# abacusorg/abacusutils

Hardware: AMD Instinct MI355X
Metric: halos/sec HOD populate (higher is better)
Workload: dtype f64; 1 GPU; C2: 1e+07 synthetic halos + 1e+07 subsample particles per GPU (seed 600+rank), LRG HOD of tests/abacus_hod.yaml:31-47, rsd=True, catalog resident in HBM; n_halo=10000000, n_part=10000000, n_gal=107980, enable_ranks=False

## Files before the change

abacusutils_amd/csrc/hod.hip:

```cpp
#include <cmath>
#include <cstring>
#include <cstddef>
#include <vector>

#include "../../include/abacus_hip.h"
#include "common.hpp"
#include "hod_classify.hpp"
#include "hod_envelope.hpp"

namespace abacus {
int exclusive_scan_u32(unsigned int *counters, int64_t n, int64_t *out, DevBuf &scratch, int zero_counters);
int sort_pairs_u16(const unsigned short *keys_in, unsigned short *keys_out, const unsigned int *val_in, unsigned int *val_out,
                   int64_t n, DevBuf &tmp);
}
using namespace abacus;

namespace {

constexpr int TILE = 2048;
constexpr int BLOCK = 256;
constexpr int PER_THREAD = TILE / BLOCK;
constexpr int SB_TILES_SPARSE = 16, SB_TILES_DENSE = 8;
constexpr int SB_TILES_MIN = 8, SB_TILES_MAX = 16;

// ... 739 lines not shown
    asm volatile("global_load_dwordx4 %0, %1, off" : "=v"(dst) : "v"(p) : "memory");
}
__device__ __forceinline__ void aload_u16(unsigned int &dst, const void *p) {
    asm volatile("global_load_ushort %0, %1, off" : "=v"(dst) : "v"(p) : "memory");
}
__device__ __forceinline__ void aload_i8(int &dst, const void *p) {
    asm volatile("global_load_sbyte %0, %1, off" : "=v"(dst) : "v"(p) : "memory");
}
template <int K>
__device__ __forceinline__ void await_vm() {
    asm volatile("s_waitcnt vmcnt(%0)" ::"n"(K) : "memory");
}
__device__ __forceinline__ void touch4(v4u &a) { asm volatile("" : "+v"(a)); }
__device__ __forceinline__ void touch1(unsigned int &a) { asm volatile("" : "+v"(a)); }
__device__ __forceinline__ void touch1i(int &a) { asm volatile("" : "+v"(a)); }

struct ExactCand {
    double mass, w, rnd, dc, fe, sh, r0, r1, r2, r3;
    long long pinds;
    int q, loc;
};

__device__ __forceinline__ void fetch_cand(const HodPtrs &a, const abacus_hod_params &p, bool sat, int64_t i, bool need_ranks,
                                           bool need_conf, ExactCand &c) {
    c.r0 = c.r1 = c.r2 = c.r3 = 1.0;
    c.pinds = 0;
    if (!sat) {
        if (a.hrec) {
            const HaloRec &r = a.hrec[i];
            c.mass = r.mass, c.w = r.multis, c.rnd = r.rnd, c.dc = r.deltac, c.fe = r.fenv, c.sh = p.want_ELG ? r.shear : 0.0;
        } else {
            c.rnd = a.hrandoms[i];
            c.mass = a.hmass[i], c.w = a.hmultis[i], c.dc = load1(a.hdeltac, i, 0.0), c.fe = load1(a.hfenv, i, 0.0),
            c.sh = p.want_ELG ? load1(a.hshear, i, 0.0) : 0.0;
        }
    } else {
        if (a.prec) {
            const PartRec &r = a.prec[i];
            c.mass = r.mass, c.w = r.weights, c.rnd = r.rnd, c.dc = r.deltac, c.fe = r.fenv, c.sh = p.want_ELG ? r.shear : 0.0;
            if (need_ranks) c.r0 = r.rank0, c.r1 = r.rank1, c.r2 = r.rank2, c.r3 = r.rank3;
            if (need_conf) c.pinds = r.pinds;
        } else {
            if (need_conf) c.pinds = a.pinds[i];
            c.rnd = a.prandoms[i];
            c.mass = a.phmass[i], c.w = a.pweights[i], c.dc = load1(a.pdeltac, i, 0.0), c.fe = load1(a.pfenv, i, 0.0),
            c.sh = p.want_ELG ? load1(a.pshear, i, 0.0) : 0.0;
            if (need_ranks) c.r0 = a.pranks[i], c.r1 = a.pranksv[i], c.r2 = a.pranksp[i], c.r3 = a.pranksr[i];
        }
    }
}

template <int lane>
__device__ __forceinline__ unsigned int writelane_u32(unsigned int v, unsigned int old) {
#if defined(__HIP_DEVICE_COMPILE__)
    asm("v_writelane_b32 %0, %1, %2" : "+v"(old) : "s"(v), "n"(lane));
#endif
    return old;
}

template <int XB, bool PIPE, int SBT, int SRC = 0, bool MASKS = true>
__device__ __forceinline__ void hod_exact_body(const HodPtrs &a, int first_sb, const abacus_hod_params &p, const SatPre &pre,
                                               const abacus_cls::ClsConst &cc, int use_cls, int clear_prev,
                                               const SbIndex *sx = nullptr) {
    static_assert(SRC == 0 || (!PIPE && XB >= 128 && SBT * TILE <= 65536), "the key index feeds the plain form");
    static_assert(SRC == 1 || MASKS, "only the key index form may leave the keep masks alone");
    constexpr int SB_TILES = SBT, SB_OBJ = SBT * TILE, SB_WORDS = SB_OBJ / 32;
    constexpr int WORDS_PER_THREAD = SB_WORDS / XB;
    static_assert(SB_WORDS % XB == 0 && XB <= 512 && SB_OBJ <= 65536, "bitmap words must divide over the workgroup");
    __shared__ ExactLds<SBT> L;
    __shared__ abacus_hod_params s_p;
    __shared__ SatPre s_pre;
    const int tid = threadIdx.x;
    static_assert(sizeof(abacus_hod_params) % 8 == 0 && sizeof(SatPre) % 8 == 0, "copied as 8-byte words");
    if (tid < (int)(sizeof(abacus_hod_params) / 8))
        reinterpret_cast<unsigned long long *>(&s_p)[tid] = reinterpret_cast<const unsigned long long *>(&p)[tid];
    if (tid < (int)(sizeof(SatPre) / 8))
        reinterpret_cast<unsigned long long *>(&s_pre)[tid] = reinterpret_cast<const unsigned long long *>(&pre)[tid];
    const int g = (int)blockIdx.x + first_sb;
    const bool sat = g >= a.nsb_c;
    const int S = sat ? g - a.nsb_c : g;
// ... 73 lines not shown
            int lo = 0, hi = SBX_BINS - 1;
            while (lo < hi) {
                const int mid = (lo + hi + 1) >> 1;
                if (s_bpre[mid] <= j) lo = mid;
                else hi = mid - 1;
            }
            const int l = ((sat ? sx->sidx_s : sx->sidx_c) + obj_first)[(int)s_bstart[lo] + (j - s_bpre[lo])];
            q = l / TILE, loc = l % TILE;
        } else {
            q = exact_find_tile(L, j);
            loc = queue[(int64_t)(tile_first + q) * TILE + (j - L.pre[q])];
        }
    };
    auto fetch = [&](int q, int loc, ExactCand &c) {
        c.q = q, c.loc = loc;
        fetch_cand(a, p, sat, (int64_t)(tile_first + q) * TILE + loc, need_ranks, need_conf, c);
    };
    auto classify = [&](const ExactCand &c, int kc) {
        if (!use_cls) return -1;
        return sat ? abacus_cls::sat_classify(cc, c.mass, c.w, c.rnd, c.dc, c.fe, c.sh, c.r0, c.r1, c.r2, c.r3, kc)
                   : abacus_cls::cent_classify(cc, c.mass, c.w, c.rnd, c.dc, c.fe, c.sh);
    };
    auto exact_chain = [&](const ExactCand &c, int kc) {
        return sat ? sat_decide_cold(&s_p, &s_pre, c.mass, c.w, c.rnd, c.dc, c.fe, c.sh, c.r0, c.r1, c.r2, c.r3, kc)
                   : cent_decide_cold(&s_p, c.mass, c.w, c.rnd, c.dc, c.fe, c.sh);
    };
    auto record = [&](const ExactCand &c, int kk) {
        if (kk) {
            if constexpr (MASKS) (sat ? a.keep_s : a.keep_c)[(int64_t)(tile_first + c.q) * TILE + c.loc] = (int8_t)kk;
            const int ls = c.q * TILE + c.loc;
            atomicOr(&L.bm[kk - 1][ls >> 5], 1u << (ls & 31));
// ... 7 lines not shown
            fetch(q, loc, c);
            const int kc = need_conf ? a.keep_c[c.pinds] : 0;
            int kk = classify(c, kc);
            if (kk < 0) kk = exact_chain(c, kc);
            record(c, kk);
        }
    } else {
        const char *rec = sat ? reinterpret_cast<const char *>(a.prec) : reinterpret_cast<const char *>(a.hrec);
        const int64_t rb = sat ? (int64_t)sizeof(PartRec) : (int64_t)sizeof(HaloRec);
        auto queue_addr = [&](int jj, int &q) {
            jj = min(jj, total - 1);
            q = exact_find_tile(L, jj);
            return queue + ((int64_t)(tile_first + q) * TILE + (jj - L.pre[q]));
        };
        auto rec_addr = [&](int q, int loc) { return rec + ((int64_t)(tile_first + q) * TILE + loc) * rb; };
        auto decode = [&](const v4u (&r)[6], int q, int loc, ExactCand &c) {
            auto dbl = [](unsigned int lo, unsigned int hi) { return __hiloint2double((int)hi, (int)lo); };
            c.q = q, c.loc = loc;
            c.mass = dbl(r[0].x, r[0].y), c.w = dbl(r[0].z, r[0].w), c.rnd = dbl(r[1].x, r[1].y), c.dc = dbl(r[1].z, r[1].w);
            c.fe = dbl(r[2].x, r[2].y), c.sh = p.want_ELG ? dbl(r[2].z, r[2].w) : 0.0;
            c.r0 = c.r1 = c.r2 = c.r3 = 1.0;
            c.pinds = 0;
            if (sat) {
                if (need_ranks) c.r0 = dbl(r[3].x, r[3].y), c.r1 = dbl(r[3].z, r[3].w), c.r2 = dbl(r[4].x, r[4].y), c.r3 = dbl(r[4].z, r[4].w);
                c.pinds = (long long)(((unsigned long long)r[5].y << 32) | r[5].x);
            }
        };
        if (total > 0) {
            int j = tid;
            int q0, q1, q2;
            unsigned int loc0, loc1, loc2 = 0;
            v4u raw[6];
            aload_u16(loc0, queue_addr(j, q0));
            aload_u16(loc1, queue_addr(j + XB, q1));
            await_vm<0>();
            touch1(loc0), touch1(loc1);
            {
                const char *r0 = rec_addr(q0, (int)loc0);
#pragma unroll
                for (int l = 0; l < 6; l++)
                    if (l < 3 || sat) aload16(raw[l], r0 + 16 * l);
            }
            await_vm<0>();
#pragma unroll
            for (int l = 0; l < 6; l++)
                if (l < 3 || sat) touch4(raw[l]);
            ExactCand cur;
            decode(raw, q0, (int)loc0, cur);
            int kc = 0;
            if (need_conf) {
                aload_i8(kc, a.keep_c + cur.pinds);
                await_vm<0>();
                touch1i(kc);
            }
#pragma unroll 1
            for (; j < total; j += XB) {
                {
                    const char *r1 = rec_addr(q1, (int)loc1);
#pragma unroll
                    for (int l = 0; l < 6; l++)
                        if (l < 3 || sat) aload16(raw[l], r1 + 16 * l);
                    aload_u16(loc2, queue_addr(j + 2 * XB, q2));
                }
                int kk = classify(cur, kc);
                if (kk < 0) {
                    await_vm<0>();
#pragma unroll
                    for (int l = 0; l < 6; l++)
                        if (l < 3 || sat) touch4(raw[l]);
                    touch1(loc2);
                    kk = exact_chain(cur, kc);
                }
                record(cur, kk);
                await_vm<0>();
#pragma unroll
                for (int l = 0; l < 6; l++)
                    if (l < 3 || sat) touch4(raw[l]);
                touch1(loc2);
                decode(raw, q1, (int)loc1, cur);
                if (need_conf) {
                    aload_i8(kc, a.keep_c + cur.pinds);
                    await_vm<0>();
                    touch1i(kc);
                }
                q1 = q2, loc1 = loc2;
            }
        }
    }
    __syncthreads();
    unsigned int wbits[3][WORDS_PER_THREAD];
    unsigned long long mine = 0;
#pragma unroll
// ... 41 lines not shown
    if (tid < 4) a.sb_counts[(int64_t)g * 4 + tid] = tid == 0 ? T0 : (tid == 1 ? T1 : (tid == 2 ? T2 : 0));
}

template <int XB, bool PIPE, int SBT>
__global__ __launch_bounds__(XB) void hod_exact(HodPtrs a, int first_sb, abacus_hod_params p, SatPre pre,
                                                abacus_cls::ClsConst cc, int use_cls, int clear_prev) {
    static_assert(PIPE, "the plain form is hod_exact_plain");
    hod_exact_body<XB, true, SBT>(a, first_sb, p, pre, cc, use_cls, clear_prev);
}
template <int XB, int SBT>
__global__ __launch_bounds__(XB) __attribute__((amdgpu_waves_per_eu(4))) void hod_exact_plain(HodPtrs a, int first_sb,
                                                                                               abacus_hod_params p, SatPre pre,
                                                                                               abacus_cls::ClsConst cc, int use_cls,
                                                                                               int clear_prev) {
    hod_exact_body<XB, false, SBT>(a, first_sb, p, pre, cc, use_cls, clear_prev);
}

template <int XB, int SBT>
__global__ __launch_bounds__(XB) void hod_exact_sbidx(HodPtrs a, abacus_hod_params p, SatPre pre, abacus_cls::ClsConst cc,
                                                      int use_cls, SbIndex sx) {
    hod_exact_body<XB, false, SBT, 1, false>(a, 0, p, pre, cc, use_cls, 0, &sx);
}
template <int XB, int SBT>
__global__ __launch_bounds__(XB) void hod_exact_sbidx_masks(HodPtrs a, abacus_hod_params p, SatPre pre, abacus_cls::ClsConst cc,
                                                            int use_cls, int clear_prev, SbIndex sx) {
    hod_exact_body<XB, false, SBT, 1, true>(a, 0, p, pre, cc, use_cls, clear_prev, &sx);
}

__global__ __launch_bounds__(256) void hod_keep_masks(int nsb_c, int nsb_s, int ntile_c, int ntile_s,
                                                      const unsigned short *__restrict__ kept_c,
// ... 151 lines not shown
template <int EBLOCK, int CS>
__device__ __forceinline__ void emit_offsets(int g, bool sat, int S, int nsb_c, int nsb_s, const int *__restrict__ sb_counts,
                                             int64_t *__restrict__ totals, int64_t (&red)[EBLOCK / 64][3], int64_t (&off)[3]) {
    int64_t v[6] = {0, 0, 0, 0, 0, 0};
    emit_offsets_sum<EBLOCK, CS>(g, sat, S, nsb_c, sb_counts, 0, v);
    emit_offsets_reduce<EBLOCK, CS>(g, sat, nsb_c, nsb_s, sb_counts, totals, red, v, off);
}

struct EmitPtrs {
    const double *hpos, *hvel, *hvdev, *hmass, *ppos, *pvel, *phvel, *phmass;
    const int64_t *hid, *phid;
    const HaloRec *hrec;
    const PartRec *prec;
};

__device__ __forceinline__ void emit_gather(const EmitPtrs &in, bool sat, int64_t i, double al, double &x, double &y, double &z,
                                            double &vx, double &vy, double &vz, double &m, int64_t &id) {
    if (!sat && in.hrec) {
        const HaloRec &r = in.hrec[i];
        x = r.pos0, y = r.pos1, z = r.pos2;
        vx = r.vel[0] + al * r.vdev[0];
        vy = r.vel[1] + al * r.vdev[1];
        vz = r.vel[2] + al * r.vdev[2];
        m = r.mass, id = r.id;
    } else if (sat && in.prec) {
        const PartRec &r = in.prec[i];
        x = r.pos[0], y = r.pos[1], z = r.pos[2];
        vx = r.hvel[0] + al * (r.vel0 - r.hvel[0]);
        vy = r.hvel[1] + al * (r.vel1 - r.hvel[1]);
        vz = r.hvel[2] + al * (r.vel2 - r.hvel[2]);
        m = r.mass2, id = r.id;
    } else if (!sat) {
        x = in.hpos[3 * i], y = in.hpos[3 * i + 1], z = in.hpos[3 * i + 2];
        vx = in.hvel[3 * i] + al * in.hvdev[3 * i];
        vy = in.hvel[3 * i + 1] + al * in.hvdev[3 * i + 1];
        vz = in.hvel[3 * i + 2] + al * in.hvdev[3 * i + 2];
        m = in.hmass[i];
        id = in.hid[i];
// ... 126 lines not shown
            asm volatile("" : "+v"(x), "+v"(y), "+v"(z), "+v"(vx), "+v"(vy), "+v"(vz), "+v"(m), "+v"(id));
            if (more) {
                issue(k1, r);
                aload_u16(k2, kept + min(e + 2 * EBLOCK, total - 1));
            }
            const bool stored = j < o.cap[t];
            emit_one(p, o, t, j, x, y, z, vx, vy, vz, m, id);
            e += EBLOCK;
            if (!more) break;
            if (__all(stored)) await_vm<8>();
            else await_vm<0>();
            touch1(k2);
            k1 = k2;
        }
        return;
    }
}

constexpr int EMIT_WIN = 2048;
constexpr int LB_VBITS = 34, LB_TAG_SHIFT = LB_VBITS + 1;
constexpr unsigned long long LB_VMASK = (1ull << LB_VBITS) - 1, LB_INCL = 1ull << LB_VBITS;
constexpr unsigned int LB_TAG_MAX = (1u << (64 - LB_TAG_SHIFT)) - 1;
constexpr int LB_PER_LANE = 8, LB_WIN = 64 * LB_PER_LANE;
constexpr int LB_SPIN = 1 << 20;
typedef __attribute__((address_space(1))) unsigned long long gu64_t;

__device__ __forceinline__ unsigned long long lb_load(const unsigned long long *w) {
    return __hip_atomic_load((gu64_t *)w, __ATOMIC_RELAXED, __HIP_MEMORY_SCOPE_AGENT);
}
__device__ __forceinline__ void lb_store(unsigned long long *w, unsigned long long v) {
// ... 537 lines not shown
    unsigned int lb_tag = 0;
    bool emit_bm = false;
    int64_t *d_totals = nullptr;
    int64_t *h_totals = nullptr;
    int64_t *h_totals_dev = nullptr;
    DevBuf out[3];
    int64_t cap[3] = {0, 0, 0};
    int64_t counts[6] = {0, 0, 0, 0, 0, 0};
    abacus_hod_params params;
    bool have_run = false, counts_valid = false;
    DevBuf shadow;
    FiltCols fc = {};
    bool shadow_ok = false, shadow_rand_ok = false;
    DevBuf hrec, prec;
    bool rec_ok = false, rec_rand_ok = false;
    HodRanges ranges;
    bool ranges_ok = false;
    DevBuf keys;
    bool keys_ok = false;
};

namespace {


struct HodOpts {
    int sbtiles, nobalance, norec, one_stage, f64filter, nokeys, nolazy, deal, noindex, nocls, pipe, eblock, dbg, sbindex, keepmasks;
};
const HodOpts &hod_opts() {
    static HodOpts o;
    static unsigned int seen = 0;
    static bool have = false;
    const unsigned int v = option_version();
    if (!have || v != seen) {
        o.sbtiles = option("hod_sbtiles"), o.nobalance = option("hod_nobalance"), o.norec = option("hod_norec");
        o.one_stage = option("hod_one_stage"), o.f64filter = option("hod_f64filter"), o.nokeys = option("hod_nokeys");
        o.nolazy = option("hod_nolazy"), o.deal = option("hod_deal"), o.noindex = option("hod_noindex");
        o.nocls = option("hod_nocls"), o.pipe = option("hod_pipe"), o.eblock = option("hod_eblock"), o.dbg = option("dbg");
        o.sbindex = option("hod_sbindex"), o.keepmasks = option("hod_keepmasks");
        seen = v, have = true;
    }
    return o;
}

template <class T>
int upload(T *&dst, const T *src, int64_t n, bool on_device) {
    if (src == nullptr) {
        dst = nullptr;
        return 0;
    }
    if (on_device) {
        dst = const_cast<T *>(src);
        return 0;
    }
// ... 12 lines not shown

OutCols out_cols(abacus_hod_state *st) {
    OutCols o;
    for (int t = 0; t < 3; t++) {
        double *base = st->out[t].as<double>();
        for (int c = 0; c < 7; c++) o.c[t][c] = base + (int64_t)c * st->cap[t];
        o.id[t] = reinterpret_cast<int64_t *>(base + (int64_t)7 * st->cap[t]);
        o.cap[t] = st->cap[t];
    }
    return o;
}

int build_records(abacus_hod_state *st) {
    const bool norec = hod_opts().norec != 0;
    if (!st->owns || norec || (st->rec_ok && st->rec_rand_ok)) return 0;
    ABACUS_TRY(st->hrec.reserve((size_t)std::max<int64_t>(st->nh, 1) * sizeof(HaloRec)));
    ABACUS_TRY(st->prec.reserve((size_t)std::max<int64_t>(st->np, 1) * sizeof(PartRec)));
    RecSrc c;
    c.hpos = st->hpos, c.hvel = st->hvel, c.hvdev = st->hveldev, c.hmass = st->hmass, c.hmultis = st->hmultis,
    c.hrandoms = st->hrandoms, c.hdeltac = st->hdeltac, c.hfenv = st->hfenv, c.hshear = st->hshear, c.hid = st->hid;
    c.ppos = st->ppos, c.pvel = st->pvel, c.phvel = st->phvel, c.phmass = st->phmass, c.pweights = st->pweights,
    c.prandoms = st->prandoms, c.pdeltac = st->pdeltac, c.pfenv = st->pfenv, c.pshear = st->pshear, c.phid = st->phid;
    c.pinds = st->pinds;
    c.pranks[0] = st->pranks, c.pranks[1] = st->pranksv, c.pranks[2] = st->pranksp, c.pranks[3] = st->pranksr;
    const int grid = (int)std::min<int64_t>(std::max<int64_t>(ceil_div(std::max(st->nh, st->np), 256), 1), 8192);
    if (!st->rec_ok)
        ABACUS_LAUNCH("hod_build_recs", hod_build_recs<false>, dim3(grid), dim3(256), 0, st->nh, st->np, c, st->hrec.as<HaloRec>(),
                      st->prec.as<PartRec>());
    else
        ABACUS_LAUNCH("hod_refresh_recs", hod_build_recs<true>, dim3(grid), dim3(256), 0, st->nh, st->np, c, st->hrec.as<HaloRec>(),
                      st->prec.as<PartRec>());
    st->rec_ok = st->rec_rand_ok = true;
    return 0;
}

HodPtrs make_ptrs(const abacus_hod_state *st) {
    HodPtrs a;
    a.nh = st->nh, a.np = st->np, a.ntile_c = st->ntile_c, a.ntile_s = st->ntile_s, a.nsb_c = st->nsb_c, a.nsb_s = st->nsb_s;
    a.hmass = st->hmass, a.hmultis = st->hmultis, a.hrandoms = st->hrandoms, a.hdeltac = st->hdeltac,
    a.hfenv = st->hfenv, a.hshear = st->hshear;
    a.phmass = st->phmass, a.pweights = st->pweights, a.prandoms = st->prandoms, a.pdeltac = st->pdeltac,
    a.pfenv = st->pfenv, a.pshear = st->pshear, a.pranks = st->pranks, a.pranksv = st->pranksv,
    a.pranksp = st->pranksp, a.pranksr = st->pranksr, a.pinds = st->pinds;
    a.keep_c = st->keep_c, a.keep_s = st->keep_s, a.q_count = st->q_count, a.queue_c = st->queue_c,
    a.queue_s = st->queue_s, a.kept_c = st->kept_c, a.kept_s = st->kept_s, a.sb_counts = st->sb_counts;
    const bool rec = st->rec_ok && st->rec_rand_ok;
    a.hrec = rec ? st->hrec.as<HaloRec>() : nullptr;
    a.prec = rec ? st->prec.as<PartRec>() : nullptr;
    return a;
}

void set_superblocks(abacus_hod_state *st, const abacus_hod_params *p) {
    int sbt = hod_opts().sbtiles;
    if (sbt != SB_TILES_DENSE && sbt != SB_TILES_SPARSE) sbt = (p->want_ELG || p->want_QSO) ? SB_TILES_DENSE : SB_TILES_SPARSE;
    st->sb_tiles = sbt;
    const int per_round = 3 * 256;
    auto count = [&](int ntile) {
        int n = (int)ceil_div(ntile, sbt);
        if (sbt == SB_TILES_DENSE && n > 256 && !hod_opts().nobalance) n = (int)ceil_div(n, per_round) * per_round;
        return std::min(n, std::max(ntile, 0));
    };
    st->nsb_c = count(st->ntile_c);
    st->nsb_s = count(st->ntile_s);
}

int launch_emit(abacus_hod_state *st) {
    const int nemit = st->nsb_c + st->nsb_s;
    if (nemit == 0) {
        ABACUS_LAUNCH("hod_emit", hod_zero_totals, dim3(1), dim3(64), 0, st->h_totals_dev);
        return 0;
    }
    EmitPtrs in;
    in.hpos = st->hpos, in.hvel = st->hvel, in.hvdev = st->hveldev, in.hmass = st->hmass, in.hid = st->hid;
    in.ppos = st->ppos, in.pvel = st->pvel, in.phvel = st->phvel, in.phmass = st->phmass, in.phid = st->phid;
    const bool rec = st->rec_ok && st->rec_rand_ok;
    in.hrec = rec ? st->hrec.as<HaloRec>() : nullptr;
    in.prec = rec ? st->prec.as<PartRec>() : nullptr;
    if (st->emit_bm) {
        const int cur = st->bm_par, prev = cur ^ 1;
        unsigned int *bm = st->bm.as<unsigned int>();
        if (st->lb_n != nemit || st->lb_tag == LB_TAG_MAX) {
            const size_t bytes = (size_t)3 * nemit * sizeof(unsigned long long);
            ABACUS_TRY(st->lb.reserve(bytes));
            HIP_TRY(hipMemsetAsync(st->lb.p, 0, bytes, stream()));
            st->lb_n = nemit, st->lb_tag = 0;
        }
        static int resident = 0;
        if (!resident) {
            int dev = 0, ncu = 0, per_cu = 0;
            HIP_TRY(hipGetDevice(&dev));
            HIP_TRY(hipDeviceGetAttribute(&ncu, hipDeviceAttributeMultiprocessorCount, dev));
            HIP_TRY(hipOccupancyMaxActiveBlocksPerMultiprocessor(&per_cu, hod_emit_bm<256, SB_TILES_SPARSE>, 256, 0));
            resident = std::min(std::max(per_cu, 1), 5) * std::max(ncu, 1);
        }
        ABACUS_LAUNCH("hod_emit", (hod_emit_bm<256, SB_TILES_SPARSE>), dim3(std::min(nemit, resident)), dim3(256), 0, st->nsb_c,
                      st->nsb_s, st->ntile_c, st->ntile_s, (const unsigned int *)(bm + (int64_t)cur * 3 * st->bm_words),
                      bm + (int64_t)prev * 3 * st->bm_words, st->bm_words, st->bm_mask[cur], st->bm_mask[prev],
                      reinterpret_cast<unsigned long long *>(st->lb.p), st->lb_tag + 1, st->keep_c, st->keep_s, st->h_totals_dev,
                      in, st->params, out_cols(st));
        st->lb_tag++;
        st->bm_mask[prev] = 0;
        return 0;
    }
    int eb = hod_opts().eblock;
    if (eb != 256 && eb != 384 && eb != 512) eb = (st->params.want_ELG || st->params.want_QSO) ? 384 : 256;
#define EMIT(EB, SBT)                                                                                                       \
    ABACUS_LAUNCH("hod_emit", (hod_emit<EB, SBT>), dim3(nemit), dim3(EB), 0, st->nsb_c, st->nsb_s, st->ntile_c, st->ntile_s, st->kept_c, st->kept_s, \
                  st->sb_counts, st->h_totals_dev, in, st->params, out_cols(st), hod_opts().dbg)
    const bool sparse = st->sb_tiles == SB_TILES_SPARSE;
    if (eb == 384 && sparse) EMIT(384, SB_TILES_SPARSE);
    else if (eb == 384) EMIT(384, SB_TILES_DENSE);
    else if (eb == 256 && sparse) EMIT(256, SB_TILES_SPARSE);
    else if (eb == 256) EMIT(256, SB_TILES_DENSE);
    else if (sparse) EMIT(512, SB_TILES_SPARSE);
    else EMIT(512, SB_TILES_DENSE);
#undef EMIT
    return 0;
}

int build_keys(abacus_hod_state *st) {
    if (st->keys_ok) return 0;
    const int64_t ph = (int64_t)std::max(st->ntile_c, 1) * TILE, pp = (int64_t)std::max(st->ntile_s, 1) * TILE;
    ABACUS_TRY(st->keys.reserve((size_t)(ph + pp) * sizeof(unsigned short)));
// ... 316 lines not shown
int abacus_hod_update(abacus_hod_state *st, const char *field, const double *host) {
    ABACUS_ENTER();
    if (!st || !field || !host) return fail("abacus_hod_update: null argument");
    double *dst = nullptr;
    int64_t n = 0;
    if (!strcmp(field, "hrandoms")) dst = st->hrandoms, n = st->nh;
    else if (!strcmp(field, "hveldev")) dst = st->hveldev, n = 3 * st->nh;
    else if (!strcmp(field, "prandoms")) dst = st->prandoms, n = st->np;
    else return fail("abacus_hod_update: unknown field '%s'", field);
    if (n == 0) return 0;
    HIP_TRY(hipMemcpyAsync(dst, host, n * sizeof(double), hipMemcpyHostToDevice, stream()));
    HIP_TRY(hipStreamSynchronize(stream()));
    st->shadow_rand_ok = false;
    st->keys_ok = false;
    st->rec_rand_ok = false;
    return 0;
}

int abacus_hod_set_sigma3d(abacus_hod_state *st, const double *sigma3d, int on_device) {
    ABACUS_ENTER();
    if (!st || !sigma3d) return fail("abacus_hod_set_sigma3d: null argument");
    if (st->owns_sigma && st->hsigma3d) HIP_TRY(hipFree(st->hsigma3d));
    st->hsigma3d = nullptr;
    st->owns_sigma = false;
    if (on_device) {
        st->hsigma3d = const_cast<double *>(sigma3d);
        return 0;
    }
    HIP_TRY(hipMalloc((void **)&st->hsigma3d, (size_t)(st->nh > 0 ? st->nh : 1) * sizeof(double)));
    st->owns_sigma = true;
// ... 9 lines not shown
    if (st->nh > 0 && !st->hsigma3d) return fail("abacus_hod_reseed: hsigma3d has not been set (abacus_hod_set_sigma3d)");
    if (halo_index0 < 0 || part_index0 < 0) return fail("abacus_hod_reseed: negative index offset");
    if (st->nh > 0) {
        const int grid = (int)std::min<int64_t>(ceil_div(st->nh, 256), 256 * 32);
        ABACUS_LAUNCH("hod_reseed_halos", hod_reseed_halos, dim3(grid), dim3(256), 0, st->nh, halo_index0,
                      (unsigned long long)seed, st->hsigma3d, want_expvel, st->hrandoms, st->hveldev);
    }
    if (st->np > 0) {
        const int grid = (int)std::min<int64_t>(ceil_div(ceil_div(st->np, 4) + 1, 256), 256 * 32);
        ABACUS_LAUNCH("hod_reseed_particles", hod_reseed_particles, dim3(grid), dim3(256), 0, st->np, part_index0,
                      (unsigned long long)seed, st->prandoms);
    }
    st->shadow_rand_ok = false;
    st->keys_ok = false;
    st->rec_rand_ok = false;
    return 0;
}

int abacus_hod_fetch_field(abacus_hod_state *st, const char *field, double *host) {
    ABACUS_ENTER();
    if (!st || !field || !host) return fail("abacus_hod_fetch_field: null argument");
    const double *src = nullptr;
    int64_t n = 0;
    if (!strcmp(field, "hrandoms")) src = st->hrandoms, n = st->nh;
    else if (!strcmp(field, "hveldev")) src = st->hveldev, n = 3 * st->nh;
    else if (!strcmp(field, "prandoms")) src = st->prandoms, n = st->np;
    else return fail("abacus_hod_fetch_field: unknown field '%s'", field);
    if (n == 0) return 0;
    HIP_TRY(hipMemcpyAsync(host, src, n * sizeof(double), hipMemcpyDeviceToHost, stream()));
    HIP_TRY(hipStreamSynchronize(stream()));
// ... 139 lines not shown

int abacus_hod_populate_async(abacus_hod_state *st, const abacus_hod_params *p) {
    ABACUS_ENTER();
    if (!st || !p) return fail("abacus_hod_populate: null argument");
    if (p->enable_ranks && st->np > 0 && (!st->pranks || !st->pranksv || !st->pranksp || !st->pranksr))
        return fail("abacus_hod_populate: enable_ranks set but the rank arrays were not staged");
    if (p->want_ELG && st->np > 0 && !st->pinds)
        return fail("abacus_hod_populate: ELG conformity needs pinds to be staged");
    st->params = *p;
    const SatPre pre = make_pre(p);
    Filt F = make_filter(*p, pre);
    const int need_env = (p->want_LRG && (p->L_Acent != 0 || p->L_Bcent != 0)) ||
                         (p->want_ELG && (p->E_Acent != 0 || p->E_Bcent != 0)) ||
                         (p->want_QSO && (p->Q_Acent != 0 || p->Q_Bcent != 0));
    const int need_shear = p->want_ELG && p->E_Ccent != 0 && st->hshear != nullptr;
    ABACUS_TRY(build_records(st));
    set_superblocks(st, p);
    const HodPtrs a = make_ptrs(st);
    const bool conf = p->want_ELG && st->pinds != nullptr && st->ntile_s > 0;
    const int ntile = st->ntile_c + st->ntile_s, nsb = st->nsb_c + st->nsb_s;
    const bool force64 = hod_opts().f64filter != 0;
    const bool use32 = st->owns && !force64;
    if (use32 && !st->shadow_ok) ABACUS_TRY(build_shadows(st, false));
    else if (use32 && !st->shadow_rand_ok) ABACUS_TRY(build_shadows(st, true));
    const FiltCols fc = st->fc;
    if (use32) ABACUS_TRY(compute_ranges(st));
    if (use32) ABACUS_TRY(build_keys(st));
    const Cheap cheap = use32 ? make_cheap(*p, F, st->ranges, hod_opts().one_stage != 0) : Cheap{};
    const KeyTab keytab = use32 ? make_keytab(cheap) : KeyTab{};
    const bool filter_first_ = conf && use32 && cheap.s_ok;
    const bool lazy_ok = use32 && !hod_opts().nokeys && !hod_opts().nolazy && cheap.c_ok && cheap.s_ok && st->ntile_c > 0 &&
                         st->ntile_s > 0 && (!conf || filter_first_) && st->sb_tiles == SB_TILES_SPARSE;
    const bool lazy_masks = lazy_ok && st->kept_valid && st->kept_sb_tiles == st->sb_tiles;
    const bool sbx_mix = !hod_opts().sbindex && !hod_opts().deal && !conf && use32 && !hod_opts().nokeys && !hod_opts().nolazy &&
                         cheap.c_ok && cheap.s_ok && st->sb_tiles == SB_TILES_SPARSE;
    const bool sbx_lazy = st->kept_valid && st->kept_sb_tiles == st->sb_tiles;
    st->kept_valid = false;
    const bool bm_path = !hod_opts().deal && !conf;
    const bool bm_was_valid = st->bm_valid;
// ... 18 lines not shown
                        deal.start[deal.nseg] = lo, deal.pre[deal.nseg] = pre;
                        pre += hi - lo, cand[kind] += hi - lo;
                        deal.nseg++;
                    }
                }
                if (kind == 0) deal.nseg_c = deal.nseg;
            }
            deal.pre[deal.nseg] = pre;
            if ((int64_t)pre <= (st->nh + st->np) / 8) {
                index_mode = true;
                st->last_cand[0] = cand[0], st->last_cand[1] = cand[1];
            }
        }
    }
    if (!index_mode) st->last_cand[0] = st->last_cand[1] = -1;
    if (index_mode && sbx_mix && st->sbx_ok) return populate_sbindex(st, p, pre, a, keytab, sbx_lazy);
    ABACUS_TRY(materialise_masks(st));
    if (index_mode && bm_path) return populate_bitmaps(st, p, pre, a, deal, bm_was_valid);
    const int exact_flags = (lazy_masks ? 1 : 0) | (index_mode ? 2 : 0);
    auto filter32 = [&](int first, int count) -> int {
        const int c0 = std::min(first, st->ntile_c), c1 = std::min(first + count, st->ntile_c);
        const int s0 = std::max(first, st->ntile_c) - st->ntile_c, s1 = std::max(first + count, st->ntile_c) - st->ntile_c;
#define F32(KIND, TWO, first_, count_)                                                                                \
    ABACUS_LAUNCH("hod_filter", (hod_filter32<KIND, TWO>), dim3(count_), dim3(FBLOCK), 0, a, fc, first_, p->want_LRG, \
                  p->want_ELG, p->want_QSO, p->enable_ranks, need_env, need_shear, F, cheap)
        const bool c2 = cheap.c_ok != 0, s2 = cheap.s_ok != 0;
        const bool keyed = !hod_opts().nokeys;
        const unsigned short *hk = st->keys.as<unsigned short>(), *pk = hk + (int64_t)std::max(st->ntile_c, 1) * TILE;
        const bool kc = keyed && c2 && c0 == 0 && c1 == st->ntile_c && c1 > c0, ks = keyed && s2 && s0 == 0 && s1 == st->ntile_s && s1 > s0;
        const int gc = (int)ceil_div(st->ntile_c, KEY_TILES), gs = (int)ceil_div(st->ntile_s, KEY_TILES);
#define FKEY(KIND, grid_) ABACUS_LAUNCH("hod_filter", (hod_filter_key<KIND>), dim3(grid_), dim3(FBLOCK), 0, a, hk, pk, gc, keytab, lazy_masks ? 1 : 0)
        if (kc && ks) {
            FKEY(2, gc + gs);
            return 0;
        }
        if (kc) FKEY(0, gc);
        if (ks) FKEY(1, gs);
#undef FKEY
        if (kc) {
            if (s1 > s0 && !ks) {
// ... 35 lines not shown
                              (const unsigned int *)st->index_idx.as<unsigned int>(),                                \
                              (const unsigned int *)(st->index_idx.as<unsigned int>() + st->nh), deal);             \
        } else if (use32) ABACUS_TRY(filter32(first, count));                                                               \
        else                                                                                                         \
            ABACUS_LAUNCH("hod_filter", hod_filter, dim3(count), dim3(FBLOCK), 0, a, first, p->want_LRG, p->want_ELG, \
                          p->want_QSO, p->enable_ranks, need_env, need_shear, F);                                    \
    }
    const bool nocls = hod_opts().nocls != 0 || !abacus_cls::cls_params_finite(*p);
    abacus_cls::ClsConst cc;
    abacus_cls::make_cls_const(*p, pre, cc);
    const int pipe_opt = hod_opts().pipe;
    const bool pipe = a.hrec && a.prec && (pipe_opt == 2 || (pipe_opt != 1 && (p->want_ELG || p->want_QSO)));
    const bool sparse_sb = st->sb_tiles == SB_TILES_SPARSE;
#define EXACT_(PIPE, SBT, first, count)                                                                                      \
    do {                                                                                                                     \
        if (PIPE)                                                                                                            \
            ABACUS_LAUNCH("hod_exact", (hod_exact<256, true, SBT>), dim3(count), dim3(256), 0, a, first, *p, pre, cc,        \
                          nocls ? 0 : 1, exact_flags);                                                                       \
        else                                                                                                                 \
            ABACUS_LAUNCH("hod_exact", (hod_exact_plain<256, SBT>), dim3(count), dim3(256), 0, a, first, *p, pre, cc,        \
                          nocls ? 0 : 1, exact_flags);                                                                       \
    } while (0)
#define EXACT(first, count)                                                    \
    if ((count) > 0) {                                                         \
        if (pipe && sparse_sb) EXACT_(true, SB_TILES_SPARSE, first, count);    \
        else if (pipe) EXACT_(true, SB_TILES_DENSE, first, count);             \
        else if (sparse_sb) EXACT_(false, SB_TILES_SPARSE, first, count);      \
        else EXACT_(false, SB_TILES_DENSE, first, count);                      \
    }
    const bool filter_first = conf && use32 && cheap.s_ok;
    if (!conf) {
// ... 159 lines not shown
```

abacusutils_amd/csrc/runtime.hip:

```cpp
#include <atomic>
#include <cstring>
#include <map>
#include <string>
#include <mutex>
#include <vector>

#include "../../include/abacus_hip.h"
#include <algorithm>

#include "common.hpp"

namespace abacus {

static thread_local std::string g_err;
static int g_device = 0;
static bool g_inited = false;
static hipStream_t g_stream = nullptr;
static bool g_own_stream = false;
static std::mutex g_mu;

int fail(const char *fmt, ...) {
    char buf[1024];
    va_list ap;
    va_start(ap, fmt);
// ... 170 lines not shown
    auto it = option_table().find(name);
    return it == option_table().end() ? 0 : it->second;
}

unsigned int option_version() { return g_option_version.load(std::memory_order_acquire); }

}

using namespace abacus;

extern "C" {

int abacus_set_option(const char *name, int value) {
    if (!name) return abacus::fail("abacus_set_option: null name");
    static const char *known[] = {"dbg", "dbg_fft", "dbg_tsc", "fft_fuse_small", "fft_hipfft", "fft_inplace", "gfft_dbg", "gfft_nofixed", "fft_nofuse", "hod_eblock", "hod_f64filter",
                                  "hod_deal", "hod_sbindex", "hod_keepmasks", "hod_nobalance", "hod_nocls", "hod_noindex", "hod_nokeys", "hod_nolazy", "hod_norec", "hod_one_stage", "hod_pipe", "hod_sbtiles", "pairs_countsort", "pairs_gen", "pairs_noblocks", "pairs_jk_grid", "pairs_nolut", "pk_nobatch", "pk_noxbin", "pk_noxbin_cross", "pk_noxbin_inter", "pk_xbin_gen", "pk_xbin_pairs", "prep_columnwise", "slab_nocompact", "slab_nofuse", "slab_nopackfuse", "slab_nounpackfuse", "tsc_acc64", "tsc_atomic", "tsc_lines_cfg1", "tsc_lines_clk", "tsc_lines_sync", "tsc_noshare", "tsc_noslabfast", "tsc_oldlists"};
    bool ok = false;
    for (const char *k : known) ok = ok || !strcmp(k, name);
    if (!ok) return abacus::fail("abacus_set_option: unknown option '%s'", name);
    std::lock_guard<std::recursive_mutex> guard(abacus::api_mutex());
    abacus::option_table()[name] = value;
    abacus::g_option_version.fetch_add(1, std::memory_order_release);
    return 0;
}

int abacus_get_option(const char *name) { return name ? abacus::option(name) : 0; }


const char *abacus_last_error(void) { return g_err.c_str(); }

int abacus_device_count(int *n) {
// ... 174 lines not shown
```

Before: 571.2 billion halos/s.

## Defer record rebuild after reseed and read fresh randoms from side columns

After the random columns are reseeded, packed halo and particle records are no longer rebuilt right away. The records are kept with stale random and velocity-deviation fields, and new exact and emit kernel variants read those fields from the fresh column arrays instead. The full rebuild only happens once the same randoms are used a second time, and the 32-bit shadow refresh moves inside the filter launch so it runs only when that filter path is taken. This avoids rebuilding records for randoms that are used only once, at the cost of extra scattered loads per candidate and new guard paths that fail on bitmap or key-index routes.

```diff
diff --git a/abacusutils_amd/csrc/hod.hip b/abacusutils_amd/csrc/hod.hip
--- a/abacusutils_amd/csrc/hod.hip
+++ b/abacusutils_amd/csrc/hod.hip
@@ -777,6 +777,11 @@
 __device__ __forceinline__ void touch4(v4u &a) { asm volatile("" : "+v"(a)); }
 __device__ __forceinline__ void touch1(unsigned int &a) { asm volatile("" : "+v"(a)); }
 __device__ __forceinline__ void touch1i(int &a) { asm volatile("" : "+v"(a)); }
+typedef unsigned int v2u __attribute__((ext_vector_type(2)));
+__device__ __forceinline__ void aload8(v2u &dst, const void *p) {
+    asm volatile("global_load_dwordx2 %0, %1, off" : "=v"(dst) : "v"(p) : "memory");
+}
+__device__ __forceinline__ void touch2(v2u &a) { asm volatile("" : "+v"(a)); }
 
 struct ExactCand {
     double mass, w, rnd, dc, fe, sh, r0, r1, r2, r3;
@@ -784,6 +789,7 @@
     int q, loc;
 };
 
+template <bool STALE = false>
 __device__ __forceinline__ void fetch_cand(const HodPtrs &a, const abacus_hod_params &p, bool sat, int64_t i, bool need_ranks,
                                            bool need_conf, ExactCand &c) {
     c.r0 = c.r1 = c.r2 = c.r3 = 1.0;
@@ -791,7 +797,8 @@
     if (!sat) {
         if (a.hrec) {
             const HaloRec &r = a.hrec[i];
-            c.mass = r.mass, c.w = r.multis, c.rnd = r.rnd, c.dc = r.deltac, c.fe = r.fenv, c.sh = p.want_ELG ? r.shear : 0.0;
+            c.mass = r.mass, c.w = r.multis, c.rnd = STALE ? a.hrandoms[i] : r.rnd, c.dc = r.deltac, c.fe = r.fenv,
+            c.sh = p.want_ELG ? r.shear : 0.0;
         } else {
             c.rnd = a.hrandoms[i];
             c.mass = a.hmass[i], c.w = a.hmultis[i], c.dc = load1(a.hdeltac, i, 0.0), c.fe = load1(a.hfenv, i, 0.0),
@@ -800,7 +807,8 @@
     } else {
         if (a.prec) {
             const PartRec &r = a.prec[i];
-            c.mass = r.mass, c.w = r.weights, c.rnd = r.rnd, c.dc = r.deltac, c.fe = r.fenv, c.sh = p.want_ELG ? r.shear : 0.0;
+            c.mass = r.mass, c.w = r.weights, c.rnd = STALE ? a.prandoms[i] : r.rnd, c.dc = r.deltac, c.fe = r.fenv,
+            c.sh = p.want_ELG ? r.shear : 0.0;
             if (need_ranks) c.r0 = r.rank0, c.r1 = r.rank1, c.r2 = r.rank2, c.r3 = r.rank3;
             if (need_conf) c.pinds = r.pinds;
         } else {
@@ -821,12 +829,13 @@
     return old;
 }
 
-template <int XB, bool PIPE, int SBT, int SRC = 0, bool MASKS = true>
+template <int XB, bool PIPE, int SBT, int SRC = 0, bool MASKS = true, bool STALE = false>
 __device__ __forceinline__ void hod_exact_body(const HodPtrs &a, int first_sb, const abacus_hod_params &p, const SatPre &pre,
                                                const abacus_cls::ClsConst &cc, int use_cls, int clear_prev,
                                                const SbIndex *sx = nullptr) {
     static_assert(SRC == 0 || (!PIPE && XB >= 128 && SBT * TILE <= 65536), "the key index feeds the plain form");
     static_assert(SRC == 1 || MASKS, "only the key index form may leave the keep masks alone");
+    static_assert(SRC == 0 || !STALE, "the key index forms read fresh records");
     constexpr int SB_TILES = SBT, SB_OBJ = SBT * TILE, SB_WORDS = SB_OBJ / 32;
     constexpr int WORDS_PER_THREAD = SB_WORDS / XB;
     static_assert(SB_WORDS % XB == 0 && XB <= 512 && SB_OBJ <= 65536, "bitmap words must divide over the workgroup");
@@ -930,7 +939,7 @@
     };
     auto fetch = [&](int q, int loc, ExactCand &c) {
         c.q = q, c.loc = loc;
-        fetch_cand(a, p, sat, (int64_t)(tile_first + q) * TILE + loc, need_ranks, need_conf, c);
+        fetch_cand<STALE>(a, p, sat, (int64_t)(tile_first + q) * TILE + loc, need_ranks, need_conf, c);
     };
     auto classify = [&](const ExactCand &c, int kc) {
         if (!use_cls) return -1;
@@ -968,6 +977,9 @@
             return queue + ((int64_t)(tile_first + q) * TILE + (jj - L.pre[q]));
         };
         auto rec_addr = [&](int q, int loc) { return rec + ((int64_t)(tile_first + q) * TILE + loc) * rb; };
+        const double *rnd_col = sat ? a.prandoms : a.hrandoms;
+        auto rnd_addr = [&](int q, int loc) { return rnd_col + ((int64_t)(tile_first + q) * TILE + loc); };
+        v2u rr = {0u, 0u};
         auto decode = [&](const v4u (&r)[6], int q, int loc, ExactCand &c) {
             auto dbl = [](unsigned int lo, unsigned int hi) { return __hiloint2double((int)hi, (int)lo); };
             c.q = q, c.loc = loc;
@@ -975,6 +987,7 @@
             c.fe = dbl(r[2].x, r[2].y), c.sh = p.want_ELG ? dbl(r[2].z, r[2].w) : 0.0;
             c.r0 = c.r1 = c.r2 = c.r3 = 1.0;
             c.pinds = 0;
+            if constexpr (STALE) c.rnd = dbl(rr.x, rr.y);
             if (sat) {
                 if (need_ranks) c.r0 = dbl(r[3].x, r[3].y), c.r1 = dbl(r[3].z, r[3].w), c.r2 = dbl(r[4].x, r[4].y), c.r3 = dbl(r[4].z, r[4].w);
                 c.pinds = (long long)(((unsigned long long)r[5].y << 32) | r[5].x);
@@ -994,11 +1007,13 @@
 #pragma unroll
                 for (int l = 0; l < 6; l++)
                     if (l < 3 || sat) aload16(raw[l], r0 + 16 * l);
+                if constexpr (STALE) aload8(rr, rnd_addr(q0, (int)loc0));
             }
             await_vm<0>();
 #pragma unroll
             for (int l = 0; l < 6; l++)
                 if (l < 3 || sat) touch4(raw[l]);
+            if constexpr (STALE) touch2(rr);
             ExactCand cur;
             decode(raw, q0, (int)loc0, cur);
             int kc = 0;
@@ -1014,6 +1029,7 @@
 #pragma unroll
                     for (int l = 0; l < 6; l++)
                         if (l < 3 || sat) aload16(raw[l], r1 + 16 * l);
+                    if constexpr (STALE) aload8(rr, rnd_addr(q1, (int)loc1));
                     aload_u16(loc2, queue_addr(j + 2 * XB, q2));
                 }
                 int kk = classify(cur, kc);
@@ -1022,6 +1038,7 @@
 #pragma unroll
                     for (int l = 0; l < 6; l++)
                         if (l < 3 || sat) touch4(raw[l]);
+                    if constexpr (STALE) touch2(rr);
                     touch1(loc2);
                     kk = exact_chain(cur, kc);
                 }
@@ -1030,6 +1047,7 @@
 #pragma unroll
                 for (int l = 0; l < 6; l++)
                     if (l < 3 || sat) touch4(raw[l]);
+                if constexpr (STALE) touch2(rr);
                 touch1(loc2);
                 decode(raw, q1, (int)loc1, cur);
                 if (need_conf) {
@@ -1101,6 +1119,12 @@
                                                                                                abacus_cls::ClsConst cc, int use_cls,
                                                                                                int clear_prev) {
     hod_exact_body<XB, false, SBT>(a, first_sb, p, pre, cc, use_cls, clear_prev);
+}
+
+template <int XB, bool PIPE, int SBT>
+__global__ __launch_bounds__(XB) void hod_exact_stale(HodPtrs a, int first_sb, abacus_hod_params p, SatPre pre,
+                                                      abacus_cls::ClsConst cc, int use_cls, int clear_prev) {
+    hod_exact_body<XB, PIPE, SBT, 0, true, true>(a, first_sb, p, pre, cc, use_cls, clear_prev);
 }
 
 template <int XB, int SBT>
@@ -1282,14 +1306,15 @@
     const PartRec *prec;
 };
 
+template <bool STALE = false>
 __device__ __forceinline__ void emit_gather(const EmitPtrs &in, bool sat, int64_t i, double al, double &x, double &y, double &z,
                                             double &vx, double &vy, double &vz, double &m, int64_t &id) {
     if (!sat && in.hrec) {
         const HaloRec &r = in.hrec[i];
         x = r.pos0, y = r.pos1, z = r.pos2;
-        vx = r.vel[0] + al * r.vdev[0];
-        vy = r.vel[1] + al * r.vdev[1];
-        vz = r.vel[2] + al * r.vdev[2];
+        vx = r.vel[0] + al * (STALE ? in.hvdev[3 * i] : r.vdev[0]);
+        vy = r.vel[1] + al * (STALE ? in.hvdev[3 * i + 1] : r.vdev[1]);
+        vz = r.vel[2] + al * (STALE ? in.hvdev[3 * i + 2] : r.vdev[2]);
         m = r.mass, id = r.id;
     } else if (sat && in.prec) {
         const PartRec &r = in.prec[i];
@@ -1446,6 +1471,40 @@
             k1 = k2;
         }
         return;
+    }
+}
+
+template <int EBLOCK, int SBT>
+__global__ __launch_bounds__(EBLOCK) void hod_emit_stale(int nsb_c, int nsb_s, int ntile_c, int ntile_s,
+                                                         const unsigned short *__restrict__ kept_c,
+                                                         const unsigned short *__restrict__ kept_s,
+                                                         const int *__restrict__ sb_counts, int64_t *__restrict__ totals,
+                                                         EmitPtrs in, abacus_hod_params p, OutCols o_arg) {
+    __shared__ int64_t red[EBLOCK / 64][3];
+    __shared__ OutCols o;
+    const int tid = threadIdx.x;
+    if (tid < (int)(sizeof(OutCols) / 8))
+        reinterpret_cast<unsigned long long *>(&o)[tid] = reinterpret_cast<const unsigned long long *>(&o_arg)[tid];
+    const int g = blockIdx.x;
+    const bool sat = g >= nsb_c;
+    const int S = sat ? g - nsb_c : g;
+    const int64_t obj_first = (int64_t)sb_first_tile(S, sat ? ntile_s : ntile_c, sat ? nsb_s : nsb_c) * TILE;
+    int64_t off[3];
+    const unsigned short *kept = (sat ? kept_s : kept_c) + obj_first;
+    const double a0 = sat ? p.L_alpha_s : p.L_alpha_c, a1 = sat ? p.E_alpha_s : p.E_alpha_c,
+                 a2 = sat ? p.Q_alpha_s : p.Q_alpha_c;
+    emit_offsets<EBLOCK, 4>(g, sat, S, nsb_c, nsb_s, sb_counts, totals, red, off);
+    const int m0 = sb_counts[(int64_t)g * 4], m1 = sb_counts[(int64_t)g * 4 + 1], m2 = sb_counts[(int64_t)g * 4 + 2];
+    const int total = m0 + m1 + m2;
+    const int64_t off0 = off[0], off1 = off[1], off2 = off[2];
+    for (int e = tid; e < total; e += EBLOCK) {
+        const int t = e < m0 ? 0 : (e < m0 + m1 ? 1 : 2);
+        const int64_t j = t == 0 ? off0 + e : (t == 1 ? off1 + (e - m0) : off2 + (e - m0 - m1));
+        const double al = t == 0 ? a0 : (t == 1 ? a1 : a2);
+        double x, y, z, vx, vy, vz, m;
+        int64_t id;
+        emit_gather<true>(in, sat, obj_first + kept[e], al, x, y, z, vx, vy, vz, m, id);
+        emit_one(p, o, t, j, x, y, z, vx, vy, vz, m, id);
     }
 }
 
@@ -2013,6 +2072,7 @@
     bool shadow_ok = false, shadow_rand_ok = false;
     DevBuf hrec, prec;
     bool rec_ok = false, rec_rand_ok = false;
+    int rand_uses = 0;
     HodRanges ranges;
     bool ranges_ok = false;
     DevBuf keys;
@@ -2024,6 +2084,7 @@
 
 struct HodOpts {
     int sbtiles, nobalance, norec, one_stage, f64filter, nokeys, nolazy, deal, noindex, nocls, pipe, eblock, dbg, sbindex, keepmasks;
+    int eager_refresh;
 };
 const HodOpts &hod_opts() {
     static HodOpts o;
@@ -2035,7 +2096,7 @@
         o.one_stage = option("hod_one_stage"), o.f64filter = option("hod_f64filter"), o.nokeys = option("hod_nokeys");
         o.nolazy = option("hod_nolazy"), o.deal = option("hod_deal"), o.noindex = option("hod_noindex");
         o.nocls = option("hod_nocls"), o.pipe = option("hod_pipe"), o.eblock = option("hod_eblock"), o.dbg = option("dbg");
-        o.sbindex = option("hod_sbindex"), o.keepmasks = option("hod_keepmasks");
+        o.sbindex = option("hod_sbindex"), o.keepmasks = option("hod_keepmasks"), o.eager_refresh = option("hod_eager_refresh");
         seen = v, have = true;
     }
     return o;
@@ -2078,6 +2139,7 @@
 int build_records(abacus_hod_state *st) {
     const bool norec = hod_opts().norec != 0;
     if (!st->owns || norec || (st->rec_ok && st->rec_rand_ok)) return 0;
+    if (st->rec_ok && st->rand_uses < 2 && !hod_opts().eager_refresh) return 0;
     ABACUS_TRY(st->hrec.reserve((size_t)std::max<int64_t>(st->nh, 1) * sizeof(HaloRec)));
     ABACUS_TRY(st->prec.reserve((size_t)std::max<int64_t>(st->np, 1) * sizeof(PartRec)));
     RecSrc c;
@@ -2098,6 +2160,9 @@
     return 0;
 }
 
+bool recs_used(const abacus_hod_state *st) { return st->owns && st->rec_ok && !hod_opts().norec; }
+bool recs_stale(const abacus_hod_state *st) { return recs_used(st) && !st->rec_rand_ok; }
+
 HodPtrs make_ptrs(const abacus_hod_state *st) {
     HodPtrs a;
     a.nh = st->nh, a.np = st->np, a.ntile_c = st->ntile_c, a.ntile_s = st->ntile_s, a.nsb_c = st->nsb_c, a.nsb_s = st->nsb_s;
@@ -2108,7 +2173,7 @@
     a.pranksp = st->pranksp, a.pranksr = st->pranksr, a.pinds = st->pinds;
     a.keep_c = st->keep_c, a.keep_s = st->keep_s, a.q_count = st->q_count, a.queue_c = st->queue_c,
     a.queue_s = st->queue_s, a.kept_c = st->kept_c, a.kept_s = st->kept_s, a.sb_counts = st->sb_counts;
-    const bool rec = st->rec_ok && st->rec_rand_ok;
+    const bool rec = recs_used(st);
     a.hrec = rec ? st->hrec.as<HaloRec>() : nullptr;
     a.prec = rec ? st->prec.as<PartRec>() : nullptr;
     return a;
@@ -2137,10 +2202,11 @@
     EmitPtrs in;
     in.hpos = st->hpos, in.hvel = st->hvel, in.hvdev = st->hveldev, in.hmass = st->hmass, in.hid = st->hid;
     in.ppos = st->ppos, in.pvel = st->pvel, in.phvel = st->phvel, in.phmass = st->phmass, in.phid = st->phid;
-    const bool rec = st->rec_ok && st->rec_rand_ok;
+    const bool rec = recs_used(st), stale = recs_stale(st);
     in.hrec = rec ? st->hrec.as<HaloRec>() : nullptr;
     in.prec = rec ? st->prec.as<PartRec>() : nullptr;
     if (st->emit_bm) {
+        if (stale) return fail("hod_emit: the bitmap emission was handed records with stale random fields");
         const int cur = st->bm_par, prev = cur ^ 1;
         unsigned int *bm = st->bm.as<unsigned int>();
         if (st->lb_n != nemit || st->lb_tag == LB_TAG_MAX) {
@@ -2169,8 +2235,14 @@
     int eb = hod_opts().eblock;
     if (eb != 256 && eb != 384 && eb != 512) eb = (st->params.want_ELG || st->params.want_QSO) ? 384 : 256;
 #define EMIT(EB, SBT)                                                                                                       \
-    ABACUS_LAUNCH("hod_emit", (hod_emit<EB, SBT>), dim3(nemit), dim3(EB), 0, st->nsb_c, st->nsb_s, st->ntile_c, st->ntile_s, st->kept_c, st->kept_s, \
-                  st->sb_counts, st->h_totals_dev, in, st->params, out_cols(st), hod_opts().dbg)
+    do {                                                                                                                    \
+        if (stale)                                                                                                          \
+            ABACUS_LAUNCH("hod_emit", (hod_emit_stale<EB, SBT>), dim3(nemit), dim3(EB), 0, st->nsb_c, st->nsb_s, st->ntile_c, st->ntile_s, st->kept_c, st->kept_s, \
+                          st->sb_counts, st->h_totals_dev, in, st->params, out_cols(st));                                   \
+        else                                                                                                                \
+            ABACUS_LAUNCH("hod_emit", (hod_emit<EB, SBT>), dim3(nemit), dim3(EB), 0, st->nsb_c, st->nsb_s, st->ntile_c, st->ntile_s, st->kept_c, st->kept_s, \
+                          st->sb_counts, st->h_totals_dev, in, st->params, out_cols(st), hod_opts().dbg);                   \
+    } while (0)
     const bool sparse = st->sb_tiles == SB_TILES_SPARSE;
     if (eb == 384 && sparse) EMIT(384, SB_TILES_SPARSE);
     else if (eb == 384) EMIT(384, SB_TILES_DENSE);
@@ -2517,6 +2589,7 @@
     st->shadow_rand_ok = false;
     st->keys_ok = false;
     st->rec_rand_ok = false;
+    st->rand_uses = 0;
     return 0;
 }
 
@@ -2556,6 +2629,7 @@
     st->shadow_rand_ok = false;
     st->keys_ok = false;
     st->rec_rand_ok = false;
+    st->rand_uses = 0;
     return 0;
 }
 
@@ -2725,15 +2799,16 @@
                          (p->want_ELG && (p->E_Acent != 0 || p->E_Bcent != 0)) ||
                          (p->want_QSO && (p->Q_Acent != 0 || p->Q_Bcent != 0));
     const int need_shear = p->want_ELG && p->E_Ccent != 0 && st->hshear != nullptr;
+    if (st->rand_uses < 2) st->rand_uses++;
     ABACUS_TRY(build_records(st));
     set_superblocks(st, p);
     const HodPtrs a = make_ptrs(st);
+    const bool stale = recs_stale(st);
     const bool conf = p->want_ELG && st->pinds != nullptr && st->ntile_s > 0;
     const int ntile = st->ntile_c + st->ntile_s, nsb = st->nsb_c + st->nsb_s;
     const bool force64 = hod_opts().f64filter != 0;
     const bool use32 = st->owns && !force64;
     if (use32 && !st->shadow_ok) ABACUS_TRY(build_shadows(st, false));
-    else if (use32 && !st->shadow_rand_ok) ABACUS_TRY(build_shadows(st, true));
     const FiltCols fc = st->fc;
     if (use32) ABACUS_TRY(compute_ranges(st));
     if (use32) ABACUS_TRY(build_keys(st));
@@ -2782,6 +2857,7 @@
         }
     }
     if (!index_mode) st->last_cand[0] = st->last_cand[1] = -1;
+    if (index_mode && stale) return fail("abacus_hod_populate: the key index path was reached with stale record fields");
     if (index_mode && sbx_mix && st->sbx_ok) return populate_sbindex(st, p, pre, a, keytab, sbx_lazy);
     ABACUS_TRY(materialise_masks(st));
     if (index_mode && bm_path) return populate_bitmaps(st, p, pre, a, deal, bm_was_valid);
@@ -2789,9 +2865,12 @@
     auto filter32 = [&](int first, int count) -> int {
         const int c0 = std::min(first, st->ntile_c), c1 = std::min(first + count, st->ntile_c);
         const int s0 = std::max(first, st->ntile_c) - st->ntile_c, s1 = std::max(first + count, st->ntile_c) - st->ntile_c;
-#define F32(KIND, TWO, first_, count_)                                                                                \
-    ABACUS_LAUNCH("hod_filter", (hod_filter32<KIND, TWO>), dim3(count_), dim3(FBLOCK), 0, a, fc, first_, p->want_LRG, \
-                  p->want_ELG, p->want_QSO, p->enable_ranks, need_env, need_shear, F, cheap)
+#define F32(KIND, TWO, first_, count_)                                                                                    \
+    do {                                                                                                                  \
+        if (!st->shadow_rand_ok) ABACUS_TRY(build_shadows(st, true));                                                     \
+        ABACUS_LAUNCH("hod_filter", (hod_filter32<KIND, TWO>), dim3(count_), dim3(FBLOCK), 0, a, fc, first_, p->want_LRG, \
+                      p->want_ELG, p->want_QSO, p->enable_ranks, need_env, need_shear, F, cheap);                         \
+    } while (0)
         const bool c2 = cheap.c_ok != 0, s2 = cheap.s_ok != 0;
         const bool keyed = !hod_opts().nokeys;
         const unsigned short *hk = st->keys.as<unsigned short>(), *pk = hk + (int64_t)std::max(st->ntile_c, 1) * TILE;
@@ -2857,7 +2936,10 @@
     const bool sparse_sb = st->sb_tiles == SB_TILES_SPARSE;
 #define EXACT_(PIPE, SBT, first, count)                                                                                      \
     do {                                                                                                                     \
-        if (PIPE)                                                                                                            \
+        if (stale)                                                                                                           \
+            ABACUS_LAUNCH("hod_exact", (hod_exact_stale<256, PIPE, SBT>), dim3(count), dim3(256), 0, a, first, *p, pre, cc,  \
+                          nocls ? 0 : 1, exact_flags);                                                                       \
+        else if (PIPE)                                                                                                       \
             ABACUS_LAUNCH("hod_exact", (hod_exact<256, true, SBT>), dim3(count), dim3(256), 0, a, first, *p, pre, cc,        \
                           nocls ? 0 : 1, exact_flags);                                                                       \
         else                                                                                                                 \
diff --git a/abacusutils_amd/csrc/runtime.hip b/abacusutils_amd/csrc/runtime.hip
--- a/abacusutils_amd/csrc/runtime.hip
+++ b/abacusutils_amd/csrc/runtime.hip
@@ -208,7 +208,7 @@
 int abacus_set_option(const char *name, int value) {
     if (!name) return abacus::fail("abacus_set_option: null name");
     static const char *known[] = {"dbg", "dbg_fft", "dbg_tsc", "fft_fuse_small", "fft_hipfft", "fft_inplace", "gfft_dbg", "gfft_nofixed", "fft_nofuse", "hod_eblock", "hod_f64filter",
-                                  "hod_deal", "hod_sbindex", "hod_keepmasks", "hod_nobalance", "hod_nocls", "hod_noindex", "hod_nokeys", "hod_nolazy", "hod_norec", "hod_one_stage", "hod_pipe", "hod_sbtiles", "pairs_countsort", "pairs_gen", "pairs_noblocks", "pairs_jk_grid", "pairs_nolut", "pk_nobatch", "pk_noxbin", "pk_noxbin_cross", "pk_noxbin_inter", "pk_xbin_gen", "pk_xbin_pairs", "prep_columnwise", "slab_nocompact", "slab_nofuse", "slab_nopackfuse", "slab_nounpackfuse", "tsc_acc64", "tsc_atomic", "tsc_lines_cfg1", "tsc_lines_clk", "tsc_lines_sync", "tsc_noshare", "tsc_noslabfast", "tsc_oldlists"};
+                                  "hod_deal", "hod_eager_refresh", "hod_sbindex", "hod_keepmasks", "hod_nobalance", "hod_nocls", "hod_noindex", "hod_nokeys", "hod_nolazy", "hod_norec", "hod_one_stage", "hod_pipe", "hod_sbtiles", "pairs_countsort", "pairs_gen", "pairs_noblocks", "pairs_jk_grid", "pairs_nolut", "pk_nobatch", "pk_noxbin", "pk_noxbin_cross", "pk_noxbin_inter", "pk_xbin_gen", "pk_xbin_pairs", "prep_columnwise", "slab_nocompact", "slab_nofuse", "slab_nopackfuse", "slab_nounpackfuse", "tsc_acc64", "tsc_atomic", "tsc_lines_cfg1", "tsc_lines_clk", "tsc_lines_sync", "tsc_noshare", "tsc_noslabfast", "tsc_oldlists"};
     bool ok = false;
     for (const char *k : known) ok = ok || !strcmp(k, name);
     if (!ok) return abacus::fail("abacus_set_option: unknown option '%s'", name);
```

Result: no change. 571.1 billion halos/s (-0.0%).
